# aerius-labs/paillier-halo2

Hardware: AMD Instinct MI355X
Metric: Paillier-encrypt proofs/s (2048-bit n, k=17); MSM achieved HBM GB/s vs peak (higher is better)
Workload: dtype u32 limbs (29-bit reduced radix, 254-bit modular integers), u64 limbs (4096-bit integers)

## Files before the change

paillier_halo2_amd/csrc/pz_lookup.hip:

```cpp
#include "fp.cuh"
#include "pz_internal.h"

int pz_batch_invert_internal(pz_ctx* ctx, Fr* d_a, size_t n, Fr* d_mul_io);
int pz_prefix_product_batch_internal(pz_ctx* ctx, const Fr* d_a, size_t a_stride, size_t n_cols, size_t n, Fr z0, Fr* d_z,
                                     size_t z_stride);

__device__ __forceinline__ u32 small_value(const Fr& mont, u32 M) {
    Fr c = fp_from_mont(mont);
    u32 hi = 0;
#pragma unroll
    for (int k = 1; k < 8; ++k) hi |= c.v[k];
    return (hi == 0 && c.v[0] < M) ? c.v[0] : 0xffffffffu;
}
__device__ __forceinline__ Fr fr_small(u32 v) {
    Fr x = fp_zero<FrTag>();
    if (!v) return x;
    x.v[0] = v;
    return fp_to_mont(x);
}

__global__ __launch_bounds__(256) void k_lk_hist(const Fr* __restrict__ cols, size_t cs, size_t rows, u32 M,
                                                 u32* __restrict__ counts, u32* __restrict__ flags) {
    const size_t i = (size_t)blockIdx.x * blockDim.x + threadIdx.x;
    if (i >= rows) return;
    const u32 v = small_value(fp_load<FrTag>(cols + (size_t)blockIdx.y * cs + i), M);
    if (v == 0xffffffffu) atomicOr(flags, 1u);
    else atomicAdd(counts + (size_t)blockIdx.y * M + v, 1u);
}

__global__ __launch_bounds__(256) void k_lk_scan(const u32* __restrict__ cA, const u32* __restrict__ cS, u32 M,
                                                 u32* __restrict__ oA, u32* __restrict__ dr, u32* __restrict__ oL,
                                                 u32* __restrict__ flags) {
    __shared__ u32 s_a[256], s_d[256], s_l[256];
    const size_t col = blockIdx.x;
    const u32* a = cA + col * M;
    const u32 per = (M + 255) / 256, lo = threadIdx.x * per;
    u32 ta = 0, td = 0, tl = 0;
    bool missing = false;
    for (u32 k = 0; k < per; ++k) {
        const u32 v = lo + k;
        if (v < M) {
            const u32 ca = a[v], cs = cS[v], present = ca ? 1u : 0u;
            if (present > cs) missing = true;
            ta += ca;
            td += present;
            tl += cs - (present <= cs ? present : cs);
        }
    }
    if (missing) atomicOr(flags, 2u);
    s_a[threadIdx.x] = ta; s_d[threadIdx.x] = td; s_l[threadIdx.x] = tl;
    __syncthreads();
    if (threadIdx.x == 0) {
        u32 ra = 0, rd = 0, rl = 0;
        for (int k = 0; k < 256; ++k) {
            u32 x = s_a[k]; s_a[k] = ra; ra += x;
            x = s_d[k]; s_d[k] = rd; rd += x;
            x = s_l[k]; s_l[k] = rl; rl += x;
        }
    }
    __syncthreads();
    ta = s_a[threadIdx.x]; td = s_d[threadIdx.x]; tl = s_l[threadIdx.x];
    for (u32 k = 0; k < per; ++k) {
        const u32 v = lo + k;
        if (v < M) {
            const u32 ca = a[v], cs = cS[v], present = ca ? 1u : 0u;
            oA[col * (M + 1) + v] = ta;
            dr[col * M + v] = td;
            oL[col * (M + 1) + v] = tl;
            ta += ca;
            td += present;
            tl += cs - (present <= cs ? present : cs);
        }
    }
    if (threadIdx.x == 255) {
        oA[col * (M + 1) + M] = ta;
        oL[col * (M + 1) + M] = tl;
    }
}

__device__ __forceinline__ u32 run_of(const u32* __restrict__ off, u32 M, u32 i) {
    u32 lo = 0, hi = M;
    while (hi - lo > 1) {
        const u32 mid = (lo + hi) >> 1;
        if (off[mid] <= i) lo = mid; else hi = mid;
    }
    return lo;
}

__global__ __launch_bounds__(256) void k_lk_emit(const u32* __restrict__ oA, const u32* __restrict__ dr,
                                                 const u32* __restrict__ oL, u32 M, size_t rows, Fr* __restrict__ pin,
                                                 Fr* __restrict__ ptab, size_t os) {
    const size_t i = (size_t)blockIdx.x * blockDim.x + threadIdx.x;
    if (i >= rows) return;
    const size_t col = blockIdx.y;
    const u32* offA = oA + col * (M + 1);
    const u32 v = run_of(offA, M, (u32)i);
    const Fr fv = fr_small(v);
    fp_store(pin + col * os + i, fv);
    if (offA[v] == (u32)i) {
        fp_store(ptab + col * os + i, fv);
    } else {
        const u32 r = (u32)i - dr[col * M + v] - 1;
        fp_store(ptab + col * os + i, fr_small(run_of(oL + col * (M + 1), M, r)));
    }
}

extern "C" int pz_lookup_permute_dev(pz_ctx* ctx, const uint64_t* d_inputs, size_t n_cols, size_t col_stride,
                                     const uint64_t* d_table, size_t rows, uint32_t value_bits, uint64_t* d_perm_inputs,
                                     uint64_t* d_perm_tables, size_t out_stride) {
    if (!ctx || value_bits == 0 || value_bits > 24 || col_stride % 4 || out_stride % 4) return PZ_ERR_INVALID;
    if (n_cols && rows && (!d_inputs || !d_table || !d_perm_inputs || !d_perm_tables)) return PZ_ERR_INVALID;
    if (n_cols > 1 && (col_stride < 4 * rows || out_stride < 4 * rows)) return PZ_ERR_INVALID;
    if (n_cols == 0 || rows == 0) return PZ_OK;
    if (n_cols > 65535 || rows > 0xfffffff0u) return PZ_ERR_INVALID;
    PZ_ENTER(ctx);
    const u32 M = 1u << value_bits;
    const size_t words = n_cols * (size_t)M + M + 2 * n_cols * (size_t)(M + 1) + n_cols * (size_t)M + 4;
    void* ws;
    PZCHK(pz_ws_get(ctx, WS_BIG_C, words * 4, &ws));
    u32* cA = (u32*)ws;
    u32* cS = cA + n_cols * (size_t)M;
    u32* oA = cS + M;
    u32* dr = oA + n_cols * (size_t)(M + 1);
    u32* oL = dr + n_cols * (size_t)M;
    u32* flags = oL + n_cols * (size_t)(M + 1);
    HIPCHK(ctx, hipMemsetAsync(cA, 0, (n_cols + 1) * (size_t)M * 4, ctx->stream));
    HIPCHK(ctx, hipMemsetAsync(flags, 0, 16, ctx->stream));
    hipLaunchKernelGGL(k_lk_hist, dim3(pz_div_up(rows, 256), (unsigned)n_cols), dim3(256), 0, ctx->stream,
                       (const Fr*)d_inputs, col_stride / 4, rows, M, cA, flags);
    hipLaunchKernelGGL(k_lk_hist, dim3(pz_div_up(rows, 256), 1), dim3(256), 0, ctx->stream, (const Fr*)d_table, (size_t)0,
                       rows, M, cS, flags);
    hipLaunchKernelGGL(k_lk_scan, dim3((unsigned)n_cols), dim3(256), 0, ctx->stream, (const u32*)cA, (const u32*)cS, M, oA,
                       dr, oL, flags);
    HIPCHK(ctx, hipGetLastError());
    u32 f = 0;
    HIPCHK(ctx, hipMemcpyAsync(&f, flags, 4, hipMemcpyDeviceToHost, ctx->stream));
    HIPCHK(ctx, hipStreamSynchronize(ctx->stream));
    if (f) return PZ_ERR_RANGE;
    hipLaunchKernelGGL(k_lk_emit, dim3(pz_div_up(rows, 256), (unsigned)n_cols), dim3(256), 0, ctx->stream, (const u32*)oA,
                       (const u32*)dr, (const u32*)oL, M, rows, (Fr*)d_perm_inputs, (Fr*)d_perm_tables, out_stride / 4);
    HIPCHK(ctx, hipGetLastError());
    return PZ_OK;
}

__global__ __launch_bounds__(256) void k_lk_terms(const Fr* __restrict__ A, size_t as, const Fr* __restrict__ S,
                                                  const Fr* __restrict__ Ap, size_t aps, const Fr* __restrict__ Sp, size_t sps,
                                                  size_t n, Fr beta, Fr gamma, Fr* __restrict__ num, Fr* __restrict__ den) {
    const size_t i = (size_t)blockIdx.x * blockDim.x + threadIdx.x;
    if (i >= n) return;
    const size_t k = blockIdx.y;
    fp_store(num + k * n + i, fp_mul(fp_add(fp_load<FrTag>(A + k * as + i), beta), fp_add(fp_load<FrTag>(S + i), gamma)));
    fp_store(den + k * n + i, fp_mul(fp_add(fp_load<FrTag>(Ap + k * aps + i), beta), fp_add(fp_load<FrTag>(Sp + k * sps + i), gamma)));
}

extern "C" int pz_lookup_product_dev(pz_ctx* ctx, const uint64_t* d_inputs, size_t input_stride, const uint64_t* d_table,
                                     const uint64_t* d_perm_inputs, size_t perm_input_stride, const uint64_t* d_perm_tables,
                                     size_t perm_table_stride, size_t n_lookups, size_t n, const uint64_t beta[4],
                                     const uint64_t gamma[4], const uint64_t z0[4], uint64_t* d_z, size_t z_stride) {
    if (!ctx || !beta || !gamma || !z0 || (n && n_lookups && (!d_inputs || !d_table || !d_perm_inputs || !d_perm_tables || !d_z)))
        return PZ_ERR_INVALID;
    if (input_stride % 4 || perm_input_stride % 4 || perm_table_stride % 4 || z_stride % 4 || n_lookups > 65535) return PZ_ERR_INVALID;
    if (n_lookups > 1 && (input_stride < 4 * n || perm_input_stride < 4 * n || perm_table_stride < 4 * n || z_stride < 4 * n))
        return PZ_ERR_INVALID;
    if (!n || !n_lookups) return PZ_OK;
    PZ_ENTER(ctx);
    void* ws;
    PZCHK(pz_ws_get(ctx, WS_BIG_C, 2 * n_lookups * n * 32, &ws));
    Fr* num = (Fr*)ws;
    Fr* den = num + n_lookups * n;
    Fr b, g, z;
    memcpy(b.v, beta, 32);
    memcpy(g.v, gamma, 32);
    memcpy(z.v, z0, 32);
    hipLaunchKernelGGL(k_lk_terms, dim3(pz_div_up(n, 256), (unsigned)n_lookups), dim3(256), 0, ctx->stream, (const Fr*)d_inputs,
                       input_stride / 4, (const Fr*)d_table, (const Fr*)d_perm_inputs, perm_input_stride / 4,
                       (const Fr*)d_perm_tables, perm_table_stride / 4, n, b, g, num, den);
    HIPCHK(ctx, hipGetLastError());
    PZCHK(pz_batch_invert_internal(ctx, den, n_lookups * n, num));
    return pz_prefix_product_batch_internal(ctx, num, n, n_lookups, n, z, (Fr*)d_z, z_stride / 4);
}
```

paillier_halo2_amd/csrc/pz_quotient.hip:

```cpp
#include "fp29.cuh"
#include "pz_internal.h"

static inline Fr fp_one_host() {
    static const uint64_t ONE[4] = {0xac96341c4ffffffbULL, 0x36fc76959f60cd29ULL, 0x666ea36f7879462eULL, 0x0e0a77c19a07df2fULL};
    Fr r;
    memcpy(r.v, ONE, 32);
    return r;
}
static inline Fr fr_from_u64(const uint64_t x[4]) {
    Fr r;
    memcpy(r.v, x, 32);
    return r;
}

typedef F29<FrTag> Fr29;
__device__ __forceinline__ Fr29 fr29_c261(const Fr& c) { return f29_to_261(f29_from_fp(c)); }
__device__ __forceinline__ Fr29 fr29_one256() {
    Fr29 r;
#pragma unroll
    for (int i = 0; i < 9; ++i) r.v[i] = P29<FrTag>::R256(i);
    return r;
}

struct S29 {
    u32 v[9];
};
static bool host_fr_canonical(const uint64_t c[4]) {
    static const uint64_t R[4] = {0x43e1f593f0000001ULL, 0x2833e84879b97091ULL, 0xb85045b68181585dULL, 0x30644e72e131a029ULL};
    for (int i = 3; i >= 0; --i)
        if (c[i] != R[i]) return c[i] < R[i];
    return false;
}
static S29 host_fr_shl(const uint64_t c[4], unsigned k) {
    static const uint64_t R[4] = {0x43e1f593f0000001ULL, 0x2833e84879b97091ULL, 0xb85045b68181585dULL, 0x30644e72e131a029ULL};
    uint64_t x[4] = {c[0], c[1], c[2], c[3]};
    for (unsigned t = 0; t < k; ++t) {
        for (int i = 3; i > 0; --i) x[i] = (x[i] << 1) | (x[i - 1] >> 63);
        x[0] <<= 1;
        bool ge = true;
        for (int i = 3; i >= 0; --i)
            if (x[i] != R[i]) { ge = x[i] > R[i]; break; }
        if (ge) {
            unsigned __int128 br = 0;
            for (int i = 0; i < 4; ++i) {
                const unsigned __int128 d = (unsigned __int128)x[i] - R[i] - br;
                x[i] = (uint64_t)d;
                br = (d >> 64) & 1;
            }
        }
    }
    S29 r;
    for (int i = 0; i < 9; ++i) {
        const unsigned bit = 29u * i, j = bit >> 6, o = bit & 63;
        uint64_t w = x[j] >> o;
        if (o > 35 && j + 1 < 4) w |= x[j + 1] << (64 - o);
        r.v[i] = (u32)(w & (i < 8 ? 0x1fffffffull : 0xffffffffull));
    }
    return r;
}
static void host_fr_mul(const uint64_t a[4], const uint64_t b[4], uint64_t out[4]) {
    static const uint64_t R[4] = {0x43e1f593f0000001ULL, 0x2833e84879b97091ULL, 0xb85045b68181585dULL, 0x30644e72e131a029ULL};
    const uint64_t INV = 0xc2e1f593efffffffULL;
    uint64_t t[6] = {0, 0, 0, 0, 0, 0};
    for (int i = 0; i < 4; ++i) {
        unsigned __int128 c = 0;
        for (int j = 0; j < 4; ++j) {
            c += (unsigned __int128)a[j] * b[i] + t[j];
            t[j] = (uint64_t)c;
            c >>= 64;
        }
        c += t[4];
        t[4] = (uint64_t)c;
        t[5] = (uint64_t)(c >> 64);
        const uint64_t m = t[0] * INV;
        c = ((unsigned __int128)m * R[0] + t[0]) >> 64;
        for (int j = 1; j < 4; ++j) {
            c += (unsigned __int128)m * R[j] + t[j];
            t[j - 1] = (uint64_t)c;
            c >>= 64;
        }
        c += t[4];
        t[3] = (uint64_t)c;
        t[4] = t[5] + (uint64_t)(c >> 64);
    }
    bool ge = t[4] != 0;
    if (!ge) {
        ge = true;
        for (int i = 3; i >= 0; --i)
            if (t[i] != R[i]) { ge = t[i] > R[i]; break; }
    }
    if (ge) {
        unsigned __int128 br = 0;
        for (int i = 0; i < 4; ++i) {
            const unsigned __int128 d = (unsigned __int128)t[i] - R[i] - br;
            t[i] = (uint64_t)d;
            br = (d >> 64) & 1;
        }
    }
    memcpy(out, t, 32);
}
static void host_fr_pow(const uint64_t a[4], unsigned e, uint64_t out[4]) {
    static const uint64_t ONE[4] = {0xac96341c4ffffffbULL, 0x36fc76959f60cd29ULL, 0x666ea36f7879462eULL, 0x0e0a77c19a07df2fULL};
    uint64_t acc[4], sq[4];
    memcpy(acc, ONE, 32);
    memcpy(sq, a, 32);
    for (; e; e >>= 1) {
        if (e & 1) host_fr_mul(acc, sq, acc);
        host_fr_mul(sq, sq, sq);
    }
    memcpy(out, acc, 32);
}
extern "C" int pzx_host_selftest(void) {
    static const uint64_t ONE[4] = {0xac96341c4ffffffbULL, 0x36fc76959f60cd29ULL, 0x666ea36f7879462eULL, 0x0e0a77c19a07df2fULL};
    auto limbs_of = [](const uint64_t x[4]) { return host_fr_shl(x, 0); };
    auto same = [](const S29& a, const S29& b) { return memcmp(a.v, b.v, sizeof a.v) == 0; };
    uint64_t two[4], acc[4], pw[4];
    {
        const S29 d = host_fr_shl(ONE, 1);
        unsigned __int128 carry = 0;
        memset(two, 0, sizeof two);
        for (int i = 0; i < 9; ++i) {
            const unsigned bit = 29u * i, j = bit >> 6, o = bit & 63;
            two[j] |= (uint64_t)d.v[i] << o;
            if (o > 35 && j + 1 < 4) two[j + 1] |= (uint64_t)d.v[i] >> (64 - o);
        }
        (void)carry;
    }
    if (!same(limbs_of(two), host_fr_shl(ONE, 1))) return 1;
    host_fr_mul(ONE, ONE, acc);
    if (memcmp(acc, ONE, 32)) return 2;
    memcpy(acc, ONE, 32);
    for (unsigned k = 1; k <= 300; ++k) {
        host_fr_mul(acc, two, acc);
        if (!same(limbs_of(acc), host_fr_shl(ONE, k))) return 100 + (int)k;
        if (k % 37 == 0 || k == 300) {
            host_fr_pow(two, k, pw);
            if (memcmp(pw, acc, 32)) return 1000 + (int)k;
        }
    }
    return 0;
}
extern "C" void pzx_host_fr_mul(const uint64_t a[4], const uint64_t b[4], uint64_t out[4]) { host_fr_mul(a, b, out); }
extern "C" void pzx_host_fr_pow(const uint64_t a[4], unsigned e, uint64_t out[4]) { host_fr_pow(a, e, out); }
extern "C" void pzx_host_fr_shl(const uint64_t c[4], unsigned k, uint32_t out[9]) {
    const S29 r = host_fr_shl(c, k);
    memcpy(out, r.v, sizeof r.v);
}
__device__ __forceinline__ Fr29 f29_add_s(const Fr29& a, const u32 (&b)[9]) {
    Fr29 r;
#pragma unroll
    for (int i = 0; i < 9; ++i) r.v[i] = a.v[i] + b[i];
    return r;
// ... 87 lines not shown
    fp_store(excl + (size_t)blockIdx.y * nb * 256 + t, w);
    if (threadIdx.x == 255) f29_store_product(block_tot + (size_t)blockIdx.y * nb + blockIdx.x, f29_to_256(p));
}
__global__ void k_pp_blocks(Fr* __restrict__ block_tot, unsigned nb, size_t n_cols, Fr z0) {
    const size_t col = (size_t)blockIdx.x * blockDim.x + threadIdx.x;
    if (col >= n_cols) return;
    Fr* bt = block_tot + col * nb;
    Fr run = z0;
    for (unsigned b = 0; b < nb; ++b) {
        Fr t = fp_load<FrTag>(bt + b);
        fp_store(bt + b, run);
        run = fp_mul(run, t);
    }
}
__global__ __launch_bounds__(256) void k_pp_apply(const Fr* __restrict__ a, size_t as, size_t n, const Fr* __restrict__ excl,
                                                  const Fr* __restrict__ block_tot, unsigned nb, Fr* __restrict__ z, size_t zs) {
    a += (size_t)blockIdx.y * as;
    z += (size_t)blockIdx.y * zs;
    const size_t t = (size_t)blockIdx.x * 256 + threadIdx.x;
    const size_t lo = t * PP_K;
    if (lo >= n) return;
    Fr29 cur = f29_mul(f29_load<FrTag>(block_tot + (size_t)blockIdx.y * nb + blockIdx.x),
                       f29_load<FrTag>(excl + (size_t)blockIdx.y * nb * 256 + t));
    for (unsigned j = 0; j < PP_K && lo + j < n; ++j) {
        const Fr v = fp_load<FrTag>(a + lo + j);
        f29_store_product(z + lo + j, cur);
        cur = f29_mul(cur, f29_from_fp_shl5(v));
    }
}

int pz_prefix_product_batch_internal(pz_ctx* ctx, const Fr* d_a, size_t a_stride, size_t n_cols, size_t n, Fr z0, Fr* d_z,
                                     size_t z_stride) {
    if (!n || !n_cols) return PZ_OK;
    if (n_cols > 65535) return PZ_ERR_INVALID;
    const unsigned nb = pz_div_up(pz_div_up(n, PP_K), 256);
    void* ws;
    PZCHK(pz_ws_get(ctx, WS_BIG_B, n_cols * ((size_t)nb * 256 + nb) * 32, &ws));
    Fr* excl = (Fr*)ws;
    Fr* tot = excl + n_cols * (size_t)nb * 256;
    hipLaunchKernelGGL(k_pp_local, dim3(nb, (unsigned)n_cols), dim3(256), 0, ctx->stream, d_a, a_stride, n, excl, tot, nb);
    hipLaunchKernelGGL(k_pp_blocks, dim3(pz_div_up(n_cols, 64)), dim3(64), 0, ctx->stream, tot, nb, n_cols, z0);
    hipLaunchKernelGGL(k_pp_apply, dim3(nb, (unsigned)n_cols), dim3(256), 0, ctx->stream, d_a, a_stride, n, (const Fr*)excl,
                       (const Fr*)tot, nb, d_z, z_stride);
    HIPCHK(ctx, hipGetLastError());
    return PZ_OK;
}
int pz_prefix_product_internal(pz_ctx* ctx, const Fr* d_a, size_t n, Fr z0, Fr* d_z) {
    return pz_prefix_product_batch_internal(ctx, d_a, n, 1, n, z0, d_z, n);
}

extern "C" int pz_fr_prefix_product_dev(pz_ctx* ctx, const uint64_t* d_a, size_t n, const uint64_t z0[4], uint64_t* d_z) {
    if (!ctx || !z0 || (n && (!d_a || !d_z))) return PZ_ERR_INVALID;
    PZ_ENTER(ctx);
    return pz_prefix_product_internal(ctx, (const Fr*)d_a, n, fr_from_u64(z0), (Fr*)d_z);
}

__global__ __launch_bounds__(256) void k_perm_terms(const Fr* __restrict__ cols, size_t cs, const Fr* __restrict__ sigma,
                                                    size_t ss, unsigned m, size_t n, const Fr* __restrict__ wpow, Fr beta,
                                                    Fr gamma, Fr delta0, Fr delta, Fr* __restrict__ num,
                                                    Fr* __restrict__ den) {
    const size_t i = (size_t)blockIdx.x * blockDim.x + threadIdx.x;
    if (i >= n) return;
    const Fr29 g = fr29_c261(gamma), d = fr29_c261(delta), beta266 = f29_to_261(fr29_c261(beta));
    Fr29 nm = fr29_one256(), dn = nm;
    Fr29 bd = f29_mul(f29_mul(beta266, f29_from_fp(delta0)), f29_load_shl5<FrTag>(wpow + i));
    for (unsigned j = 0; j < m; ++j) {
        const Fr29 v = f29_add(f29_load_shl5<FrTag>(cols + (size_t)j * cs + i), g);
        const Fr29 sg = f29_load<FrTag>(sigma + (size_t)j * ss + i);
        nm = f29_mul(nm, f29_add(v, bd));
        dn = f29_mul(dn, f29_add(v, f29_mul(beta266, sg)));
        bd = f29_mul(bd, d);
    }
    f29_store<0>(num + i, nm);
    f29_store<0>(den + i, dn);
}

extern "C" int pz_permutation_product_dev(pz_ctx* ctx, const uint64_t* d_cols, size_t col_stride, const uint64_t* d_sigma,
                                          size_t sigma_stride, size_t m, uint32_t log_n, const uint64_t omega[4],
                                          const uint64_t beta[4], const uint64_t gamma[4], const uint64_t delta_start[4],
                                          const uint64_t delta[4], const uint64_t z0[4], uint64_t* d_z) {
    if (!ctx || !omega || !beta || !gamma || !delta_start || !delta || !z0 || !d_z || log_n > 26) return PZ_ERR_INVALID;
    if (m && (!d_cols || !d_sigma)) return PZ_ERR_INVALID;
    if (col_stride % 4 || sigma_stride % 4 || m > 65535) return PZ_ERR_INVALID;
    const size_t n = (size_t)1 << log_n;
    if (m > 1 && (col_stride < 4 * n || sigma_stride < 4 * n)) return PZ_ERR_INVALID;
    PZ_ENTER(ctx);
    void *wp, *ws;
    PZCHK(pz_get_pow_table(ctx, omega, n, &wp));
    PZCHK(pz_ws_get(ctx, WS_BIG_C, 2 * n * 32, &ws));
    Fr* num = (Fr*)ws;
    Fr* den = num + n;
    hipLaunchKernelGGL(k_perm_terms, dim3(pz_div_up(n, 256)), dim3(256), 0, ctx->stream, (const Fr*)d_cols, col_stride / 4,
                       (const Fr*)d_sigma, sigma_stride / 4, (unsigned)m, n, (const Fr*)wp, fr_from_u64(beta), fr_from_u64(gamma),
                       fr_from_u64(delta_start), fr_from_u64(delta), num, den);
    HIPCHK(ctx, hipGetLastError());
    PZCHK(pz_batch_invert_internal(ctx, den, n, num));
    return pz_prefix_product_internal(ctx, num, n, fr_from_u64(z0), (Fr*)d_z);
}

__global__ __launch_bounds__(256) void k_perm_terms_sets(const Fr* __restrict__ cols, size_t cs, const Fr* __restrict__ sigma,
                                                         size_t ss, unsigned m, unsigned chunk_len, size_t n,
                                                         const Fr* __restrict__ wpow, const Fr* __restrict__ dpow,
                                                         S29 beta266, S29 g, S29 d, Fr* __restrict__ num, Fr* __restrict__ den,
                                                         unsigned set0) {
    const size_t i = (size_t)blockIdx.x * blockDim.x + threadIdx.x;
    if (i >= n) return;
    const unsigned c0 = (set0 + blockIdx.y) * chunk_len, set = blockIdx.y;
    Fr29 nm = fr29_one256(), dn = nm;
    Fr29 bd = f29_mul(f29_mul_s(f29_load<FrTag>(dpow + c0), beta266.v), f29_load_shl5<FrTag>(wpow + i));
    Fr v_n = fp_load<FrTag>(cols + (size_t)c0 * cs + i), s_n = fp_load<FrTag>(sigma + (size_t)c0 * ss + i);
    for (unsigned c = c0; c < c0 + chunk_len && c < m; ++c) {
        const Fr29 v = f29_add_s(f29_from_fp_shl5(v_n), g.v);
        const Fr29 sg = f29_from_fp(s_n);
        const unsigned cn = (c + 1 < c0 + chunk_len && c + 1 < m) ? c + 1 : c;
        v_n = fp_load<FrTag>(cols + (size_t)cn * cs + i);
        s_n = fp_load<FrTag>(sigma + (size_t)cn * ss + i);
        nm = f29_mul(nm, f29_add(v, bd));
        dn = f29_mul(dn, f29_add(v, f29_mul_s(sg, beta266.v)));
        bd = f29_mul_s(bd, d.v);
    }
    f29_store_product(num + (size_t)set * n + i, nm);
    f29_store_product(den + (size_t)set * n + i, dn);
}
__global__ __launch_bounds__(256) void k_perm_chain(const Fr* __restrict__ z, size_t zs, unsigned n_sets, size_t u, Fr* __restrict__ mult) {
    __shared__ Fr s_p[256];
    const unsigned per = (n_sets + 255u) / 256u, lo = threadIdx.x * per, hi = lo + per < n_sets ? lo + per : n_sets;
    Fr p = fp_one<FrTag>();
    for (unsigned j = lo; j < hi; ++j) p = fp_mul(p, fp_load<FrTag>(z + (size_t)j * zs + u));
    s_p[threadIdx.x] = p;
    __syncthreads();
    for (unsigned off = 1; off < 256; off <<= 1) {
        Fr v = fp_one<FrTag>();
        if (threadIdx.x >= off) v = s_p[threadIdx.x - off];
        __syncthreads();
        if (threadIdx.x >= off) {
            p = fp_mul(v, p);
            s_p[threadIdx.x] = p;
        }
        __syncthreads();
    }
    Fr c = threadIdx.x ? s_p[threadIdx.x - 1] : fp_one<FrTag>();
    for (unsigned j = lo; j < hi; ++j) {
        fp_store(mult + j, c);
        c = fp_mul(c, fp_load<FrTag>(z + (size_t)j * zs + u));
    }
}
__global__ __launch_bounds__(256) void k_scale_sets(Fr* __restrict__ z, size_t zs, size_t n, const Fr* __restrict__ mult) {
    const size_t i = (size_t)blockIdx.x * blockDim.x + threadIdx.x;
    if (i >= n || blockIdx.y == 0) return;
    Fr* p = z + (size_t)blockIdx.y * zs + i;
    fp_store(p, fp_mul(fp_load<FrTag>(p), fp_load<FrTag>(mult + blockIdx.y)));
}

extern "C" int pz_permutation_product_sets_dev(pz_ctx* ctx, const uint64_t* d_cols, size_t col_stride, const uint64_t* d_sigma,
                                               size_t sigma_stride, size_t m, uint32_t chunk_len, uint32_t log_n,
                                               size_t usable_rows, const uint64_t omega[4], const uint64_t beta[4],
                                               const uint64_t gamma[4], const uint64_t delta[4], uint64_t* d_z,
                                               size_t z_stride) {
    if (!ctx || !d_cols || !d_sigma || !d_z || !omega || !beta || !gamma || !delta || m == 0 || chunk_len == 0 || log_n > 26)
        return PZ_ERR_INVALID;
    const size_t n = (size_t)1 << log_n;
    const size_t n_sets = (m + chunk_len - 1) / chunk_len;
    if (col_stride % 4 || sigma_stride % 4 || z_stride % 4 || usable_rows >= n || n_sets > 65535 || m > 0xffffffu) return PZ_ERR_INVALID;
    if ((m > 1 && (col_stride < 4 * n || sigma_stride < 4 * n)) || (n_sets > 1 && z_stride < 4 * n)) return PZ_ERR_INVALID;
    if (!host_fr_canonical(beta) || !host_fr_canonical(gamma) || !host_fr_canonical(delta)) return PZ_ERR_INVALID;
    PZ_ENTER(ctx);
    void *wp, *dp, *ws, *mu;
    PZCHK(pz_get_pow_table(ctx, omega, n, &wp));
    PZCHK(pz_get_pow_table(ctx, delta, m, &dp));
    size_t sb = ((size_t)4 << 30) / (2 * n * 32);
    if (sb < 1) sb = 1;
    if (sb > n_sets) sb = n_sets;
    PZCHK(pz_ws_get(ctx, WS_BIG_C, 2 * sb * n * 32, &ws));
    PZCHK(pz_ws_get(ctx, WS_MISC, n_sets * 32, &mu));
    Fr* num = (Fr*)ws;
    Fr* den = num + sb * n;
    for (size_t s0 = 0; s0 < n_sets; s0 += sb) {
        const size_t ns = n_sets - s0 < sb ? n_sets - s0 : sb;
        hipLaunchKernelGGL(k_perm_terms_sets, dim3(pz_div_up(n, 256), (unsigned)ns), dim3(256), 0, ctx->stream,
                           (const Fr*)d_cols, col_stride / 4, (const Fr*)d_sigma, sigma_stride / 4, (unsigned)m, (unsigned)chunk_len, n,
                           (const Fr*)wp, (const Fr*)dp, host_fr_shl(beta, 10), host_fr_shl(gamma, 5), host_fr_shl(delta, 5), num, den,
                           (unsigned)s0);
        HIPCHK(ctx, hipGetLastError());
        PZCHK(pz_batch_invert_internal(ctx, den, ns * n, num));
        PZCHK(pz_prefix_product_batch_internal(ctx, num, n, ns, n, fp_one_host(), (Fr*)d_z + s0 * (z_stride / 4), z_stride / 4));
    }
    if (n_sets > 1) {
        hipLaunchKernelGGL(k_perm_chain, dim3(1), dim3(256), 0, ctx->stream, (const Fr*)d_z, z_stride / 4, (unsigned)n_sets,
                           usable_rows, (Fr*)mu);
        hipLaunchKernelGGL(k_scale_sets, dim3(pz_div_up(n, 256), (unsigned)n_sets), dim3(256), 0, ctx->stream, (Fr*)d_z,
                           z_stride / 4, n, (const Fr*)mu);
        HIPCHK(ctx, hipGetLastError());
    }
    return PZ_OK;
}

__global__ __launch_bounds__(256) void k_quotient_gate(const Fr* __restrict__ adv, size_t as, const Fr* __restrict__ sel,
                                                       size_t ss, unsigned n_cols, size_t N, unsigned step, S29 y261,
                                                       Fr* __restrict__ h) {
    const size_t i = (size_t)blockIdx.x * blockDim.x + threadIdx.x;
    if (i >= N) return;
    const size_t i1 = (i + step) & (N - 1), i2 = (i + 2 * (size_t)step) & (N - 1), i3 = (i + 3 * (size_t)step) & (N - 1);
    Fr29 acc = f29_load<FrTag>(h + i);
    for (unsigned j = 0; j < n_cols; ++j) {
        const Fr* a = adv + (size_t)j * as;
        const Fr29 a0 = f29_load<FrTag>(a + i), a1 = f29_load<FrTag>(a + i1), a3 = f29_load<FrTag>(a + i3);
        const Fr29 a2 = f29_load_shl5<FrTag>(a + i2), sl = f29_load_shl5<FrTag>(sel + (size_t)j * ss + i);
        const Fr29 e = f29_sub<2, 29>(f29_add(a0, f29_mul(a1, a2)), a3);
        acc = f29_mul2_s(acc, y261.v, e, sl);
    }
    f29_store<0>(h + i, acc);
}

extern "C" int pz_quotient_gate_dev(pz_ctx* ctx, const uint64_t* d_adv_ext, size_t adv_stride, const uint64_t* d_sel_ext,
                                    size_t sel_stride, size_t n_cols, uint32_t log_ext, uint32_t rot_step,
                                    const uint64_t y[4], uint64_t* d_h) {
    if (!ctx || !y || !d_h || log_ext > 28 || (n_cols && (!d_adv_ext || !d_sel_ext))) return PZ_ERR_INVALID;
    if (adv_stride % 4 || sel_stride % 4 || n_cols > 0xffffffffu) return PZ_ERR_INVALID;
    const size_t N = (size_t)1 << log_ext;
    if (rot_step == 0 || rot_step >= N) return PZ_ERR_INVALID;
    if (n_cols > 1 && (adv_stride < 4 * N || sel_stride < 4 * N)) return PZ_ERR_INVALID;
    if (!host_fr_canonical(y)) return PZ_ERR_INVALID;
    if (n_cols == 0) return PZ_OK;
    PZ_ENTER(ctx);
    hipLaunchKernelGGL(k_quotient_gate, dim3(pz_div_up(N, 256)), dim3(256), 0, ctx->stream, (const Fr*)d_adv_ext,
                       adv_stride / 4, (const Fr*)d_sel_ext, sel_stride / 4, (unsigned)n_cols, N, (unsigned)rot_step,
                       host_fr_shl(y, 5), (Fr*)d_h);
    HIPCHK(ctx, hipGetLastError());
    return PZ_OK;
}

__global__ void k_vanishing_inv(Fr g, Fr w_ext, unsigned log_n, unsigned E, Fr* __restrict__ out) {
    const unsigned r = threadIdx.x;
    if (blockIdx.x || r >= E) return;
    Fr x = g;
    for (unsigned k = 0; k < r; ++k) x = fp_mul(x, w_ext);
    for (unsigned k = 0; k < log_n; ++k) x = fp_sqr(x);
    fp_store(out + r, fp_inv(fp_sub(x, fp_one<FrTag>())));
}
__global__ __launch_bounds__(256) void k_scale_periodic(Fr* __restrict__ h, size_t N, const Fr* __restrict__ tab,
                                                        unsigned mask) {
    const size_t i = (size_t)blockIdx.x * blockDim.x + threadIdx.x;
    if (i < N) fp_store(h + i, fp_mul(fp_load<FrTag>(h + i), fp_load<FrTag>(tab + (i & mask))));
}

extern "C" int pz_quotient_finish_dev(pz_ctx* ctx, uint64_t* d_h, uint32_t log_n, uint32_t log_e, const uint64_t coset_g[4],
                                      const uint64_t omega_ext[4]) {
    if (!ctx || !d_h || !coset_g || !omega_ext || log_e > 6 || log_n + log_e > 28) return PZ_ERR_INVALID;
    PZ_ENTER(ctx);
    const unsigned E = 1u << log_e;
    const size_t N = (size_t)1 << (log_n + log_e);
    void* tab;
    PZCHK(pz_ws_get(ctx, WS_MISC, E * 32, &tab));
    hipLaunchKernelGGL(k_vanishing_inv, dim3(1), dim3(64), 0, ctx->stream, fr_from_u64(coset_g), fr_from_u64(omega_ext),
                       (unsigned)log_n, E, (Fr*)tab);
    hipLaunchKernelGGL(k_scale_periodic, dim3(pz_div_up(N, 256)), dim3(256), 0, ctx->stream, (Fr*)d_h, N, (const Fr*)tab,
                       E - 1);
    HIPCHK(ctx, hipGetLastError());
    return PZ_OK;
}

__global__ __launch_bounds__(256) void k_mul_table_cols(Fr* __restrict__ a, size_t cs, size_t n, const Fr* __restrict__ tab) {
    const size_t i = (size_t)blockIdx.x * blockDim.x + threadIdx.x;
    if (i >= n) return;
    Fr* p = a + (size_t)blockIdx.y * cs + i;
    fp_store(p, fp_mul(fp_load<FrTag>(p), fp_load<FrTag>(tab + i)));
}

extern "C" int pz_fr_distribute_powers_dev(pz_ctx* ctx, uint64_t* d_a, size_t n_cols, size_t col_stride, size_t n,
                                           const uint64_t g[4], const uint64_t c[4]) {
    if (!ctx || !g || (n_cols && n && !d_a) || col_stride % 4 || (n_cols > 1 && col_stride < 4 * n)) return PZ_ERR_INVALID;
    if (n_cols == 0 || n == 0) return PZ_OK;
    if (n_cols > 65535) return PZ_ERR_INVALID;
    PZ_ENTER(ctx);
    void* tab;
    PZCHK(pz_get_pow_table(ctx, g, n, &tab, c));
    hipLaunchKernelGGL(k_mul_table_cols, dim3(pz_div_up(n, 256), (unsigned)n_cols), dim3(256), 0, ctx->stream, (Fr*)d_a,
                       col_stride / 4, n, (const Fr*)tab);
    HIPCHK(ctx, hipGetLastError());
    return PZ_OK;
}

#define KD_K 64u
__global__ __launch_bounds__(256) void k_kd_local(const Fr* __restrict__ a, size_t cs, size_t n, Fr x, Fr* __restrict__ L,
                                                  size_t n_chunks) {
    const size_t c = (size_t)blockIdx.x * blockDim.x + threadIdx.x;
    if (c >= n_chunks) return;
    const Fr* p = a + (size_t)blockIdx.y * cs;
    const size_t lo = c * KD_K, hi = (lo + KD_K < n ? lo + KD_K : n);
    Fr v = fp_zero<FrTag>();
    for (size_t i = hi; i-- > lo;) v = fp_add(fp_mul(v, x), fp_load<FrTag>(p + i));
    fp_store(L + (size_t)blockIdx.y * n_chunks + c, v);
}
__global__ __launch_bounds__(256) void k_kd_carry(Fr* __restrict__ L, size_t n_chunks, Fr x) {
    __shared__ Fr s_v[256], s_x[256];
    Fr* l = L + (size_t)blockIdx.x * n_chunks;
    Fr xk = x;
    for (unsigned s = 1; s < KD_K; s <<= 1) xk = fp_sqr(xk);
    const size_t per = (n_chunks + 255) / 256;
    const size_t lo = threadIdx.x * per, hi = lo + per < n_chunks ? lo + per : n_chunks;
    Fr V = fp_zero<FrTag>(), X = fp_one<FrTag>();
    for (size_t c = hi; c-- > lo && c < n_chunks;) {
        V = fp_add(fp_load<FrTag>(l + c), fp_mul(xk, V));
        X = fp_mul(X, xk);
    }
    s_v[threadIdx.x] = V;
    s_x[threadIdx.x] = X;
    __syncthreads();
    for (unsigned off = 1; off < 256; off <<= 1) {
        Fr v = s_v[threadIdx.x], xx = s_x[threadIdx.x];
        Fr uv = fp_zero<FrTag>(), ux = fp_one<FrTag>();
        const bool has = threadIdx.x + off < 256;
        if (has) { uv = s_v[threadIdx.x + off]; ux = s_x[threadIdx.x + off]; }
        __syncthreads();
        if (has) {
            s_v[threadIdx.x] = fp_add(v, fp_mul(xx, uv));
            s_x[threadIdx.x] = fp_mul(xx, ux);
        }
        __syncthreads();
    }
    Fr carry = threadIdx.x + 1 < 256 ? s_v[threadIdx.x + 1] : fp_zero<FrTag>();
    for (size_t c = hi; c-- > lo && c < n_chunks;) {
        Fr t = fp_load<FrTag>(l + c);
        fp_store(l + c, carry);
        carry = fp_add(t, fp_mul(xk, carry));
    }
}
__global__ __launch_bounds__(256) void k_kd_apply(const Fr* a, size_t cs, size_t n, Fr x,
                                                  const Fr* __restrict__ L, size_t n_chunks, Fr* q, size_t qs) {
// ... 430 lines not shown
```

Baseline: 1.435.

## Replace batch-inversion grand products with block-scan fraction products and single inversion

```diff
diff --git a/paillier_halo2_amd/csrc/pz_lookup.hip b/paillier_halo2_amd/csrc/pz_lookup.hip
--- a/paillier_halo2_amd/csrc/pz_lookup.hip
+++ b/paillier_halo2_amd/csrc/pz_lookup.hip
@@ -4,6 +4,11 @@
 int pz_batch_invert_internal(pz_ctx* ctx, Fr* d_a, size_t n, Fr* d_mul_io);
 int pz_prefix_product_batch_internal(pz_ctx* ctx, const Fr* d_a, size_t a_stride, size_t n_cols, size_t n, Fr z0, Fr* d_z,
                                      size_t z_stride);
+bool pz_gp_legacy();
+bool pz_fr_canonical_host(const uint64_t c[4]);
+int pz_gp_lookup_internal(pz_ctx* ctx, const Fr* A, size_t as, const Fr* S, const Fr* Ap, size_t aps, const Fr* Sp, size_t sps,
+                          size_t n_lookups, size_t n, const uint64_t beta[4], const uint64_t gamma[4], const uint64_t z0[4], Fr* d_z,
+                          size_t zs);
 
 __device__ __forceinline__ u32 small_value(const Fr& mont, u32 M) {
     Fr c = fp_from_mont(mont);
@@ -164,6 +169,10 @@
         return PZ_ERR_INVALID;
     if (!n || !n_lookups) return PZ_OK;
     PZ_ENTER(ctx);
+    if (!pz_gp_legacy() && pz_fr_canonical_host(beta) && pz_fr_canonical_host(gamma) && pz_fr_canonical_host(z0))
+        return pz_gp_lookup_internal(ctx, (const Fr*)d_inputs, input_stride / 4, (const Fr*)d_table, (const Fr*)d_perm_inputs,
+                                     perm_input_stride / 4, (const Fr*)d_perm_tables, perm_table_stride / 4, n_lookups, n, beta, gamma, z0,
+                                     (Fr*)d_z, z_stride / 4);
     void* ws;
     PZCHK(pz_ws_get(ctx, WS_BIG_C, 2 * n_lookups * n * 32, &ws));
     Fr* num = (Fr*)ws;
diff --git a/paillier_halo2_amd/csrc/pz_quotient.hip b/paillier_halo2_amd/csrc/pz_quotient.hip
--- a/paillier_halo2_amd/csrc/pz_quotient.hip
+++ b/paillier_halo2_amd/csrc/pz_quotient.hip
@@ -1,3 +1,5 @@
+#include <stdlib.h>
+
 #include "fp29.cuh"
 #include "pz_internal.h"
 
@@ -391,6 +393,321 @@
     fp_store(p, fp_mul(fp_load<FrTag>(p), fp_load<FrTag>(mult + blockIdx.y)));
 }
 
+#define GP_K 8u
+#define GP_ROWS (GP_K * 256u)
+
+__device__ __forceinline__ Fr gp_canon(Fr29 x) {
+    f29_cond_sub_kp<FrTag, 1>(x);
+    Fr r;
+    f29_pack(x, r.v);
+    return r;
+}
+__device__ __forceinline__ void gp_store_words(Fr* p, const Fr& a) {
+    uint4* q = reinterpret_cast<uint4*>(p);
+    q[0] = make_uint4(a.v[0], a.v[1], a.v[2], a.v[3]);
+    q[1] = make_uint4(a.v[4], a.v[5], a.v[6], a.v[7]);
+}
+__device__ __forceinline__ void gp_store_packed(Fr* p, const Fr29& x) {
+    Fr w;
+    f29_pack(x, w.v);
+    gp_store_words(p, w);
+}
+
+struct GpPermTerms {
+    const Fr *cols, *sigma, *wpow, *dpow;
+    size_t cs, ss;
+    unsigned m, chunk_len, set0;
+    S29 beta266, g, d;
+    struct State {
+        Fr29 bd0;
+        unsigned c0, c1;
+    };
+    __device__ __forceinline__ State init(unsigned set) const {
+        State s;
+        s.c0 = (set0 + set) * chunk_len;
+        s.c1 = s.c0 + chunk_len < m ? s.c0 + chunk_len : m;
+        s.bd0 = f29_mul_s(f29_load<FrTag>(dpow + s.c0), beta266.v);
+        return s;
+    }
+    __device__ __forceinline__ void row(const State& s, unsigned, size_t i, Fr29& nm, Fr29& dn) const {
+        nm = fr29_one256();
+        dn = nm;
+        Fr29 bd = f29_mul(s.bd0, f29_load_shl5<FrTag>(wpow + i));
+        Fr v_n = fp_load<FrTag>(cols + (size_t)s.c0 * cs + i), s_n = fp_load<FrTag>(sigma + (size_t)s.c0 * ss + i);
+        for (unsigned c = s.c0; c < s.c1; ++c) {
+            const Fr29 v = f29_add_s(f29_from_fp_shl5(v_n), g.v);
+            const Fr29 sg = f29_from_fp(s_n);
+            const unsigned cn = c + 1 < s.c1 ? c + 1 : c;
+            v_n = fp_load<FrTag>(cols + (size_t)cn * cs + i);
+            s_n = fp_load<FrTag>(sigma + (size_t)cn * ss + i);
+            nm = f29_mul(nm, f29_add(v, bd));
+            dn = f29_mul(dn, f29_add(v, f29_mul_s(sg, beta266.v)));
+            bd = f29_mul_s(bd, d.v);
+        }
+    }
+};
+struct GpLookTerms {
+    const Fr *A, *S, *Ap, *Sp;
+    size_t as, aps, sps;
+    S29 beta261, gamma256;
+    struct State {};
+    __device__ __forceinline__ State init(unsigned) const { return State(); }
+    __device__ __forceinline__ void row(const State&, unsigned k, size_t i, Fr29& nm, Fr29& dn) const {
+        nm = f29_mul(f29_add_s(f29_load_shl5<FrTag>(A + k * as + i), beta261.v), f29_add_s(f29_load<FrTag>(S + i), gamma256.v));
+        dn = f29_mul(f29_add_s(f29_load_shl5<FrTag>(Ap + k * aps + i), beta261.v), f29_add_s(f29_load<FrTag>(Sp + k * sps + i), gamma256.v));
+    }
+};
+
+struct GpWs {
+    Fr *texcl, *btot, *upair, *zu, *dinv, *cj, *carry;
+};
+
+template <class Terms> __global__ __launch_bounds__(256) void k_gp_terms(Terms q, size_t n, size_t u, Fr* __restrict__ num,
+                                                                         Fr* __restrict__ den, GpWs w, unsigned nb) {
+    __shared__ u32 s[2 * 9 * 256];
+    const unsigned set = blockIdx.y, tid = threadIdx.x;
+    const size_t lo = ((size_t)blockIdx.x * 256 + tid) * GP_K;
+    num += (size_t)set * n;
+    den += (size_t)set * n;
+    const bool owns_u = lo <= u && u - lo < GP_K && u < n;
+    Fr29 pn = fr29_one256(), pd = pn, un = pn, ud = pn;
+    if (lo < n) {
+        const typename Terms::State st = q.init(set);
+        for (unsigned j = 0; j < GP_K; ++j) {
+            const size_t i = lo + j;
+            if (i >= n) break;
+            Fr29 nm, dn;
+            q.row(st, set, i, nm, dn);
+            Fr wn, wd;
+            if (f29_is_zero(dn)) {
+                wn = fp_zero<FrTag>();
+                wd = fp_one<FrTag>();
+            } else {
+                wn = gp_canon(nm);
+                wd = gp_canon(dn);
+            }
+            gp_store_words(num + i, wn);
+            gp_store_words(den + i, wd);
+            if (owns_u && i == u) un = pn;
+            const Fr29 d5 = f29_from_fp_shl5(wd);
+            pn = f29_mul(pn, f29_from_fp_shl5(wn));
+            pd = f29_mul(pd, d5);
+            if (owns_u && i >= u) ud = f29_mul(ud, d5);
+        }
+    }
+    Fr29 a = f29_to_261(pn), b = f29_to_261(pd);
+#pragma unroll
+    for (int l = 0; l < 9; ++l) {
+        s[l * 256 + tid] = a.v[l];
+        s[(9 + l) * 256 + tid] = b.v[l];
+    }
+    __syncthreads();
+    for (unsigned off = 1; off < 256; off <<= 1) {
+        const bool fa = tid >= off, fb = tid + off < 256;
+        Fr29 x, y;
+        if (fa) {
+#pragma unroll
+            for (int l = 0; l < 9; ++l) x.v[l] = s[l * 256 + tid - off];
+        }
+        if (fb) {
+#pragma unroll
+            for (int l = 0; l < 9; ++l) y.v[l] = s[(9 + l) * 256 + tid + off];
+        }
+        __syncthreads();
+        if (fa) {
+            a = f29_mul(x, a);
+#pragma unroll
+            for (int l = 0; l < 9; ++l) s[l * 256 + tid] = a.v[l];
+        }
+        if (fb) {
+            b = f29_mul(b, y);
+#pragma unroll
+            for (int l = 0; l < 9; ++l) s[(9 + l) * 256 + tid] = b.v[l];
+        }
+        __syncthreads();
+    }
+    Fr29 ea = f29_one<FrTag>(), eb = ea;
+    if (tid) {
+#pragma unroll
+        for (int l = 0; l < 9; ++l) ea.v[l] = s[l * 256 + tid - 1];
+    }
+    if (tid < 255) {
+#pragma unroll
+        for (int l = 0; l < 9; ++l) eb.v[l] = s[(9 + l) * 256 + tid + 1];
+    }
+    const size_t blk = (size_t)set * nb + blockIdx.x;
+    if (lo < n) {
+        gp_store_packed(w.texcl + (blk * 256 + tid) * 2, ea);
+        gp_store_packed(w.texcl + (blk * 256 + tid) * 2 + 1, eb);
+    }
+    if (tid == 255) gp_store_words(w.btot + blk * 2, gp_canon(f29_to_256(a)));
+    if (tid == 0) gp_store_words(w.btot + blk * 2 + 1, gp_canon(f29_to_256(b)));
+    if (owns_u) {
+        gp_store_words(w.upair + (size_t)set * 2, gp_canon(f29_mul(un, ea)));
+        gp_store_words(w.upair + (size_t)set * 2 + 1, gp_canon(f29_mul(ud, eb)));
+    }
+}
+
+__global__ __launch_bounds__(64) void k_gp_sets(GpWs w, unsigned nb, unsigned bu) {
+    __shared__ Fr s_n[64], s_d[64];
+    const unsigned set = blockIdx.x, tid = threadIdx.x;
+    Fr* bt = w.btot + (size_t)set * nb * 2;
+    const unsigned per = (nb + 63u) / 64u, lo = tid * per < nb ? tid * per : nb, hi = lo + per < nb ? lo + per : nb;
+    Fr pn = fp_one<FrTag>(), pd = pn;
+    for (unsigned j = lo; j < hi; ++j) {
+        pn = fp_mul(pn, fp_load<FrTag>(bt + 2 * (size_t)j));
+        pd = fp_mul(pd, fp_load<FrTag>(bt + 2 * (size_t)j + 1));
+    }
+    s_n[tid] = pn;
+    s_d[tid] = pd;
+    __syncthreads();
+    for (unsigned off = 1; off < 64; off <<= 1) {
+        const bool fa = tid >= off, fb = tid + off < 64;
+        Fr x = pn, y = pd;
+        if (fa) x = s_n[tid - off];
+        if (fb) y = s_d[tid + off];
+        __syncthreads();
+        if (fa) {
+            pn = fp_mul(x, pn);
+            s_n[tid] = pn;
+        }
+        if (fb) {
+            pd = fp_mul(pd, y);
+            s_d[tid] = pd;
+        }
+        __syncthreads();
+    }
+    const Fr inv = fp_inv(s_d[0]);
+    Fr cn = tid ? s_n[tid - 1] : fp_one<FrTag>();
+    Fr cd = tid < 63 ? s_d[tid + 1] : fp_one<FrTag>();
+    Fr nbu = cn;
+    for (unsigned j = lo; j < hi; ++j) {
+        const Fr t = fp_load<FrTag>(bt + 2 * (size_t)j);
+        fp_store(bt + 2 * (size_t)j, cn);
+        if (j == bu) nbu = cn;
+        cn = fp_mul(cn, t);
+    }
+    for (unsigned j = hi; j-- > lo;) {
+        const Fr t = fp_load<FrTag>(bt + 2 * (size_t)j + 1);
+        fp_store(bt + 2 * (size_t)j + 1, cd);
+        if (j == bu) {
+            const Fr nex = fp_mul(nbu, fp_load<FrTag>(w.upair + (size_t)set * 2));
+            const Fr dsuf = fp_mul(cd, fp_load<FrTag>(w.upair + (size_t)set * 2 + 1));
+            fp_store(w.zu + set, fp_mul(fp_mul(nex, dsuf), inv));
+        }
+        cd = fp_mul(cd, t);
+    }
+    if (tid == 0) fp_store(w.dinv + set, inv);
+}
+
+__global__ __launch_bounds__(256) void k_gp_consts(GpWs w, unsigned ns, Fr z0, int chain, int first) {
+    __shared__ Fr s_p[256];
+    const unsigned tid = threadIdx.x;
+    const unsigned per = (ns + 255u) / 256u, lo = tid * per < ns ? tid * per : ns, hi = lo + per < ns ? lo + per : ns;
+    if (!chain) {
+        for (unsigned j = lo; j < hi; ++j) fp_store(w.cj + j, fp_mul(z0, fp_load<FrTag>(w.dinv + j)));
+        return;
+    }
+    const Fr start = first ? z0 : fp_mul(z0, fp_load<FrTag>(w.carry));
+    Fr p = fp_one<FrTag>();
+    for (unsigned j = lo; j < hi; ++j) p = fp_mul(p, fp_load<FrTag>(w.zu + j));
+    s_p[tid] = p;
+    __syncthreads();
+    for (unsigned off = 1; off < 256; off <<= 1) {
+        Fr v = p;
+        if (tid >= off) v = s_p[tid - off];
+        __syncthreads();
+        if (tid >= off) {
+            p = fp_mul(v, p);
+            s_p[tid] = p;
+        }
+        __syncthreads();
+    }
+    Fr c = tid ? fp_mul(start, s_p[tid - 1]) : start;
+    for (unsigned j = lo; j < hi; ++j) {
+        fp_store(w.cj + j, fp_mul(c, fp_load<FrTag>(w.dinv + j)));
+        c = fp_mul(c, fp_load<FrTag>(w.zu + j));
+    }
+    if (tid == 255) fp_store(w.carry, fp_mul(start, p));
+}
+
+__global__ __launch_bounds__(256) void k_gp_apply(const Fr* __restrict__ num, const Fr* __restrict__ den, size_t n, GpWs w, unsigned nb,
+                                                  Fr* __restrict__ z, size_t zs) {
+    const unsigned set = blockIdx.y, tid = threadIdx.x;
+    const size_t lo = ((size_t)blockIdx.x * 256 + tid) * GP_K;
+    if (lo >= n) return;
+    num += (size_t)set * n;
+    den += (size_t)set * n;
+    z += (size_t)set * zs;
+    const size_t blk = (size_t)set * nb + blockIdx.x;
+    const Fr* te = w.texcl + (blk * 256 + tid) * 2;
+    Fr29 f = f29_mul(f29_mul(f29_load<FrTag>(w.cj + set), f29_load_shl5<FrTag>(w.btot + blk * 2)), f29_load<FrTag>(te));
+    Fr29 sfx = f29_mul(f29_load_shl5<FrTag>(w.btot + blk * 2 + 1), f29_load<FrTag>(te + 1));
+    Fr29 d[GP_K];
+#pragma unroll
+    for (unsigned j = GP_K; j-- > 0;) {
+        if (lo + j < n) sfx = f29_mul(sfx, f29_load_shl5<FrTag>(den + lo + j));
+        d[j] = sfx;
+    }
+#pragma unroll
+    for (unsigned j = 0; j < GP_K; ++j) {
+        if (lo + j < n) {
+            f29_store_product(z + lo + j, f29_mul(f, d[j]));
+            f = f29_mul(f, f29_load_shl5<FrTag>(num + lo + j));
+        }
+    }
+}
+
+static size_t gp_ws_bytes(size_t ns, unsigned nb) { return (ns * ((size_t)nb * 256 * 2 + (size_t)nb * 2 + 5) + 1) * 32; }
+static GpWs gp_ws_carve(void* ws, size_t ns, unsigned nb) {
+    GpWs w;
+    w.texcl = (Fr*)ws;
+    w.btot = w.texcl + ns * (size_t)nb * 256 * 2;
+    w.upair = w.btot + ns * (size_t)nb * 2;
+    w.zu = w.upair + ns * 2;
+    w.dinv = w.zu + ns;
+    w.cj = w.dinv + ns;
+    w.carry = w.cj + ns;
+    return w;
+}
+template <class Terms> static int gp_batch(pz_ctx* ctx, const Terms& q, size_t n, size_t u, size_t ns, Fr* num, Fr* den, const GpWs& w,
+                                           Fr z0, bool first, Fr* d_z, size_t zs) {
+    const unsigned nb = pz_div_up(n, GP_ROWS);
+    const bool chain = u < n;
+    hipLaunchKernelGGL(k_gp_terms<Terms>, dim3(nb, (unsigned)ns), dim3(256), 0, ctx->stream, q, n, u, num, den, w, nb);
+    hipLaunchKernelGGL(k_gp_sets, dim3((unsigned)ns), dim3(64), 0, ctx->stream, w, nb, chain ? (unsigned)(u / GP_ROWS) : 0xffffffffu);
+    hipLaunchKernelGGL(k_gp_consts, dim3(1), dim3(256), 0, ctx->stream, w, (unsigned)ns, z0, chain ? 1 : 0, first ? 1 : 0);
+    hipLaunchKernelGGL(k_gp_apply, dim3(nb, (unsigned)ns), dim3(256), 0, ctx->stream, (const Fr*)num, (const Fr*)den, n, w, nb, d_z, zs);
+    HIPCHK(ctx, hipGetLastError());
+    return PZ_OK;
+}
+bool pz_gp_legacy() {
+    const char* e = getenv("PZ_GP_PATH");
+    return e && !strcmp(e, "legacy");
+}
+static size_t gp_set_batch_cap() {
+    const char* e = getenv("PZ_GP_SET_BATCH");
+    const long v = e ? atol(e) : 0;
+    return v > 0 ? (size_t)v : (size_t)-1;
+}
+bool pz_fr_canonical_host(const uint64_t c[4]) { return host_fr_canonical(c); }
+
+int pz_gp_lookup_internal(pz_ctx* ctx, const Fr* A, size_t as, const Fr* S, const Fr* Ap, size_t aps, const Fr* Sp, size_t sps,
+                          size_t n_lookups, size_t n, const uint64_t beta[4], const uint64_t gamma[4], const uint64_t z0[4], Fr* d_z,
+                          size_t zs) {
+    const unsigned nb = pz_div_up(n, GP_ROWS);
+    void *ws, *wb;
+    PZCHK(pz_ws_get(ctx, WS_BIG_C, 2 * n_lookups * n * 32, &ws));
+    PZCHK(pz_ws_get(ctx, WS_BIG_B, gp_ws_bytes(n_lookups, nb), &wb));
+    GpLookTerms q;
+    q.A = A; q.S = S; q.Ap = Ap; q.Sp = Sp;
+    q.as = as; q.aps = aps; q.sps = sps;
+    q.beta261 = host_fr_shl(beta, 5);
+    q.gamma256 = host_fr_shl(gamma, 0);
+    Fr* num = (Fr*)ws;
+    return gp_batch(ctx, q, n, n, n_lookups, num, num + n_lookups * n, gp_ws_carve(wb, n_lookups, nb), fr_from_u64(z0), true, d_z, zs);
+}
+
 extern "C" int pz_permutation_product_sets_dev(pz_ctx* ctx, const uint64_t* d_cols, size_t col_stride, const uint64_t* d_sigma,
                                                size_t sigma_stride, size_t m, uint32_t chunk_len, uint32_t log_n,
                                                size_t usable_rows, const uint64_t omega[4], const uint64_t beta[4],
@@ -408,12 +725,31 @@
     PZCHK(pz_get_pow_table(ctx, omega, n, &wp));
     PZCHK(pz_get_pow_table(ctx, delta, m, &dp));
     size_t sb = ((size_t)4 << 30) / (2 * n * 32);
+    const size_t cap = gp_set_batch_cap();
+    if (sb > cap) sb = cap;
     if (sb < 1) sb = 1;
     if (sb > n_sets) sb = n_sets;
     PZCHK(pz_ws_get(ctx, WS_BIG_C, 2 * sb * n * 32, &ws));
-    PZCHK(pz_ws_get(ctx, WS_MISC, n_sets * 32, &mu));
     Fr* num = (Fr*)ws;
     Fr* den = num + sb * n;
+    if (!pz_gp_legacy()) {
+        const unsigned nb = pz_div_up(n, GP_ROWS);
+        void* wb;
+        PZCHK(pz_ws_get(ctx, WS_BIG_B, gp_ws_bytes(sb, nb), &wb));
+        const GpWs w = gp_ws_carve(wb, sb, nb);
+        GpPermTerms q;
+        q.cols = (const Fr*)d_cols; q.sigma = (const Fr*)d_sigma; q.wpow = (const Fr*)wp; q.dpow = (const Fr*)dp;
+        q.cs = col_stride / 4; q.ss = sigma_stride / 4;
+        q.m = (unsigned)m; q.chunk_len = (unsigned)chunk_len;
+        q.beta266 = host_fr_shl(beta, 10); q.g = host_fr_shl(gamma, 5); q.d = host_fr_shl(delta, 5);
+        for (size_t s0 = 0; s0 < n_sets; s0 += sb) {
+            const size_t ns = n_sets - s0 < sb ? n_sets - s0 : sb;
+            q.set0 = (unsigned)s0;
+            PZCHK(gp_batch(ctx, q, n, usable_rows, ns, num, den, w, fp_one_host(), s0 == 0, (Fr*)d_z + s0 * (z_stride / 4), z_stride / 4));
+        }
+        return PZ_OK;
+    }
+    PZCHK(pz_ws_get(ctx, WS_MISC, n_sets * 32, &mu));
     for (size_t s0 = 0; s0 < n_sets; s0 += sb) {
         const size_t ns = n_sets - s0 < sb ? n_sets - s0 : sb;
         hipLaunchKernelGGL(k_perm_terms_sets, dim3(pz_div_up(n, 256), (unsigned)ns), dim3(256), 0, ctx->stream,
```

New measurement: 1.445, median of 5. Within noise of the previous version (+0.7%).
